# mehtas30/Software-Defined-Radio-Course-Project

Hardware: AMD Instinct MI355X
Metric: IQ Msamples/s (and x real-time) per GPU, mode-0 mono 2.4MS/s->48kS/s (higher is better)
Workload: dtype f32; 1 GPU; BASELINE configs[1]: mode-0 mono, 101-tap RF LPF + 10x decimate + FM demod + 51-tap audio LPF/5x decimate -> S16, 1 GiB synthetic u8 IQ per GPU (83,886 reference blocks), device-resident; mode=0, channels=1, rf_taps=101, stream_bytes_per_gpu=1073740800, blocks_per_gpu=83886, parallelism=streams x1 (one independent stream per GPU)

## Files before the change

### include/fmrx.h

```cpp
#ifndef FMRX_H
#define FMRX_H

#include <stddef.h>
#include <stdint.h>

#ifdef __cplusplus
extern "C" {
#endif

#define FMRX_OK 0
#define FMRX_EINVAL (-1)
#define FMRX_EHIP (-2)
#define FMRX_ENOMEM (-3)
#define FMRX_ESTATE (-4)

#define FMRX_STEREO 2
#define FMRX_MONO 1

typedef struct {
    int mode;
    int channels;
    int rf_taps;
    int bp_taps;
    int audio_taps;
// ... 256 lines not shown
int fmrx_rds_ext_init(fmrx_rds_ext* io);
int fmrx_rds_parse_blocks(fmrx_rds_ext* io, const fmrx_rds_block_rec* blocks, size_t n, uint64_t n_bits, int flush);
int fmrx_set_rds_sync(fmrx_ctx* ctx, int on);
int fmrx_rds_ext_get(const fmrx_ctx* ctx, int stream, fmrx_rds_ext* out);

int fmrx_fm_demod_arctan(fmrx_ctx* ctx, float* d_out, double* d_prev_phase, const float* d_i,
                         const float* d_q, int n);
int fmrx_estimate_psd(fmrx_ctx* ctx, const float* samples, size_t n, int freq_bins, float fs,
                      float* freq, float* psd_db);
int fmrx_psd_device(fmrx_ctx* ctx, const float* d_samples, size_t n, int freq_bins, float fs,
                    float* d_psd_db);

int fmrx_synth_host(uint64_t seed, int rf_fs, uint64_t first_pair, size_t n_pairs, uint8_t* out);
int fmrx_synth_device(fmrx_ctx* ctx, uint64_t seed, int rf_fs, uint64_t first_pair,
                      size_t n_pairs, uint8_t* d_out);
int fmrx_synth_device_streams(fmrx_ctx* ctx, const uint64_t* seeds, size_t n_seeds, int rf_fs,
                              uint64_t first_pair, size_t n_pairs, uint8_t* d_out, size_t stride_bytes);

int fmrx_test_pll_fallback(fmrx_ctx* ctx, int kind, const float* d_a, const float* d_b, size_t n,
                           float* d_out);

int fmrx_debug_mono_stamps(fmrx_ctx* ctx, unsigned long long* d_stamps, size_t n_workgroups, size_t* needed);

int fmrx_debug_pll_stats(fmrx_ctx* ctx, unsigned long long* d_counts);

int fmrx_debug_pll_redos(fmrx_ctx* ctx, unsigned* d_counts);

int fmrx_debug_stage_timing(fmrx_ctx* ctx, int op, double* ms, double* steps, long* launches, int n_kinds);

#define FMRX_KNOB_PLL_SPEC 0
#define FMRX_KNOB_PLL_SAT 1
#define FMRX_KNOB_PLL_PRED 2
#define FMRX_KNOB_PLL_PIPE 3
#define FMRX_KNOB_PLL_IDX 4
#define FMRX_KNOB_STEREO_CHUNKS 5
#define FMRX_KNOB_MONO_SPLIT 6
#define FMRX_KNOB_BPF_TILE 7
#define FMRX_KNOB_HALO_KERNEL 8
#define FMRX_KNOB_PLL_INJECT 9
#define FMRX_KNOB_PLL_PIPE_MISS 10
#define FMRX_KNOB_PLL_HINT_SKEW 11
#define FMRX_KNOB_PLL_CNT 12
#define FMRX_KNOB_PLL_STICK 13
#define FMRX_KNOB_STEREO_HEAD 14
#define FMRX_KNOB_STEREO_LEAD 15
#define FMRX_KNOB_AUDIO_DEFER 16
// ... 8 lines not shown
```

### software-defined-radio-course-project_amd/csrc/ctx.h

```cpp
#pragma once
#include <hip/hip_runtime.h>

#include <algorithm>
#include <cstdint>
#include <functional>
#include <limits>
#include <mutex>
#include <string>
#include <type_traits>
#include <utility>
#include <vector>

#include "../../include/fmrx.h"
#include "fmrx_internal.h"
#include "tuner.h"
#include "wide.h"

namespace fmrx {

int fail(int code, const char* fmt, ...);

#define HIPCHK(expr)                                                                   \
    do {                                                                               \
        hipError_t e_ = (expr);                                                        \
// ... 347 lines not shown
    HIPCHK(hipMemcpy(d.p, src, sizeof(float) * count, hipMemcpyHostToDevice));
    return 0;
}
inline size_t meter_frames(const fmrx_ctx* c, size_t n_blocks) {
    return n_blocks * c->geo.if_samples / ((size_t)kMeterWindows * (size_t)(c->geo.bp_fs / 1000));
}


int reset_state(fmrx_ctx* c);
int timing_begin(fmrx_ctx* c, hipStream_t st, TimingPair** ev);
inline int timing_end(TimingPair* ev, hipStream_t st) {
    if (ev) HIPCHK(hipEventRecord(ev->second, st));
    return 0;
}

int init_audio(fmrx_ctx* c);
int reset_audio(fmrx_ctx* c, const std::vector<float>& pll0);
int init_rds_front(fmrx_ctx* c);
int reset_rds_front(fmrx_ctx* c, const std::vector<float>& pll0);
int reset_deemph(fmrx_ctx* c);
int run_fused(fmrx_ctx* c, const uint8_t* d_iq, size_t n_blocks, int16_t* d_pcm, float* d_mono, float* d_demod,
              size_t demod_stride, int demod_hist, bool with_audio, size_t b0 = 0, size_t call_blocks = 0,
              hipStream_t st = nullptr, bool last = true);
int run_mono_audio(fmrx_ctx* c, const float* d_demod, size_t demod_stride, size_t n_if, int16_t* d_pcm, float* d_mono);
int run_stereo_audio(fmrx_ctx* c, size_t n_blocks, int16_t* d_pcm, float* d_mono, const float* src = nullptr);
int stereo_chunks(const fmrx_ctx* c, size_t n_blocks);
int run_stereo_pipelined(fmrx_ctx* c, const uint8_t* d_iq, size_t n_blocks, int16_t* d_pcm, float* d_mono, int K);
int run_rds(fmrx_ctx* c, const float* d_demod, size_t demod_stride, size_t n_if, float* d_out, float* d_nco,
            float* d_channel);
int ensure_demod(fmrx_ctx* c, size_t n_if);
int ensure_deemph_taps(fmrx_ctx* c);
inline int deemph_audio_fs(const fmrx_ctx* c) { return c->geo.if_fs / c->geo.audio_down; }

size_t rds_granule_blocks(const fmrx_ctx* c);
int check_rds_blocks(const fmrx_ctx* c, size_t n_blocks);
int init_rds_bits(fmrx_ctx* c);
int reset_rds_bits(fmrx_ctx* c);
int rds_decode_enqueue(fmrx_ctx* c, const float* d_demod, size_t demod_stride, size_t n_blocks);
int rds_decode_finish(fmrx_ctx* c);

void reset_rds_sync(fmrx_ctx* c);
int rds_sync_enqueue(fmrx_ctx* c, const uint8_t* d_bits, size_t n_bits);
int rds_sync_finish(fmrx_ctx* c);

void init_frames(fmrx_ctx* c);
int check_frame_blocks(const fmrx_ctx* c, size_t n_blocks, const char* who);
// ... 40 lines not shown
```

### software-defined-radio-course-project_amd/csrc/engine.cpp

```cpp
#include "ctx.h"

namespace fmrx {

static int grow_rows(fmrx_ctx* c, DevBuf<float>& buf, size_t& stride, size_t hist, size_t new_stride) {
    if (new_stride <= stride) return 0;
    const int ns = c->cfg.n_streams;
    DevBuf<float> nb;
    int rc = nb.ensure(new_stride * ns);
    if (rc) return rc;
    HIPCHK(hipMemsetAsync(nb.p, 0, sizeof(float) * nb.n, c->stream));
    if (buf.p) {
        HIPCHK(hipMemcpy2DAsync(nb.p, new_stride * sizeof(float), buf.p, stride * sizeof(float), hist * sizeof(float), ns,
                                hipMemcpyDeviceToDevice, c->stream));
        HIPCHK(hipStreamSynchronize(c->stream));
        buf.release();
    }
    buf = std::move(nb);
    stride = new_stride;
    return 0;
}

int init_audio(fmrx_ctx* c) {
    const fmrx_geometry_t& g = c->geo;
    const size_t ns = c->cfg.n_streams;
// ... 263 lines not shown
    L.stamps = c->diag.stamps;
    L.audio = with_audio ? 1 : 0;
    const bool fused_halo = (reinterpret_cast<uintptr_t>(L.iq) & 15) == 0 && L.stream_bytes % 16 == 0 &&
                            L.iq_stride % 16 == 0 && c->front.halo_bytes % 16 == 0 &&
                            c->knobs.halo_kernel != 1;
    L.halo_next = (last && fused_halo) ? c->front.halo.next() : nullptr;
    TimingPair* ev = nullptr;
    if ((rc = timing_begin(c, st, &ev))) return rc;
    const int st_t = (!with_audio && d_demod) ? c->diag.timer.begin(st) : -1;
    rc = launch_mono_fused(L, ns, c->geo.rf_taps, c->geo.rf_decim, c->geo.audio_up, c->geo.audio_down, c->taps.mono, st);
    c->diag.timer.end(st_t, kStFront, 0.0, st);
    if (rc != 0) return fail(rc == -1 ? FMRX_EINVAL : FMRX_EHIP, "fused kernel launch failed (%d)", rc);
    if ((rc = timing_end(ev, st))) return rc;
    if (with_audio) c->mono.stale = false;
    if (dx && (rc = run_quant_rows(c, dx, n_blocks * c->geo.audio_frames, d_pcm))) return rc;
    if (!last) return 0;
    if (!L.halo_next) {
        rc = launch_halo_update(d_iq, call_blocks * bb, c->front.halo.cur(), c->front.halo.next(),
                                c->front.halo_bytes, ns, st);
        if (rc != 0) return fail(FMRX_EHIP, "halo update failed");
    }
    c->front.halo.flip();
    return 0;
}

int run_mono_audio(fmrx_ctx* c, const float* d_demod, size_t demod_stride, size_t n_if,
                   int16_t* d_pcm, float* d_mono) {
    const int ns = c->cfg.n_streams;
    const int at = c->geo.audio_taps_total;
    const size_t na = n_if * c->geo.audio_up / c->geo.audio_down;
    PolyStreams P{};
    P.in = d_demod;
    P.in_stride = demod_stride;
    P.state = c->mono.hist.p;
    P.state_stride = c->mono.hist_len;
    P.coeff = c->taps.d_audio.p;
    P.taps = at;
    P.up = c->geo.audio_up;
    P.down = c->geo.audio_down;
    P.n_out = (int)na;
    float* dx = nullptr;
    int rc = quant_rows(c, na, d_mono, &dx);
    if (rc) return rc;
    P.out = dx ? dx : d_mono;
    P.out_stride = na;
    P.pcm = d_pcm;
// ... 220 lines not shown
```

### software-defined-radio-course-project_amd/csrc/mono_fused.hip

```cpp
#include <hip/hip_runtime.h>

#include <algorithm>
#include <cstdlib>

#include "dsp_device.h"
#include "mono_launch.h"

namespace fmrx {

namespace {

constexpr int kAudioTaps = 51;
constexpr int kAH = kAudioTaps - 1;

template <int T, int D, int AD, int NT, int R>
struct MonoCfg {
    static constexpr int S = R * D;
    static constexpr int G = (S % 4 == 2) ? 0 : 2;
    static constexpr int CIF = NT * R;
    static constexpr int P = CIF * D;
    static constexpr int H = T - 1;
    static constexpr int WH = T - 1 + D * (R - 1);
    static constexpr int slot(int b) { return b + G * (b / S); }
    static constexpr int XB = slot(H + P + 2) + 4;
    static constexpr int NLD = (P / 2 + NT - 1) / NT;
    static constexpr int LH0 = ((P - H) / 2) / NT;
    static constexpr int CAmax = (CIF + AD - 1) / AD;
    static constexpr int NG = (T + 1) / 2;
    static constexpr int na_for(int g) { return ((g * CIF + AD - 1) / AD + 1) / 2; }
    static constexpr int GA = na_for(3) <= NT ? 3 : na_for(2) <= NT ? 2 : 1;
    static constexpr int NA = na_for(GA);
    static constexpr int DX = AD * NA;
    static constexpr int DWI = DX + 50;
    static_assert(2 * DX >= GA * CIF, "every window sample has a slot");
    static_assert(T % 2 == 1, "odd tap count");
    static_assert(S % 2 == 0 && H % 2 == 0, "pair groups must stay 16-B aligned");
    static_assert(P % 2 == 0, "chunk must be whole dwords");
    static_assert(CAmax <= NT, "one audio output per thread per chunk");
};

__device__ inline uint32_t load4(const uint8_t* in, const uint8_t* halo, long long off,
                                 long long total, long long halo_bytes) {
    if (off >= 0) {
        if (off + 4 <= total) return *reinterpret_cast<const uint32_t*>(in + off);
        return 0x80808080u;
    }
    return *reinterpret_cast<const uint32_t*>(halo + (halo_bytes + off));
}

template <int K>
__device__ inline float sbyte(uint32_t w) {
    float f;
    if constexpr (K == 0)
        asm("v_cvt_f32_i32_sdwa %0, sext(%1) dst_sel:DWORD dst_unused:UNUSED_PAD src0_sel:BYTE_0" : "=v"(f) : "v"(w));
    else if constexpr (K == 1)
        asm("v_cvt_f32_i32_sdwa %0, sext(%1) dst_sel:DWORD dst_unused:UNUSED_PAD src0_sel:BYTE_1" : "=v"(f) : "v"(w));
    else if constexpr (K == 2)
        asm("v_cvt_f32_i32_sdwa %0, sext(%1) dst_sel:DWORD dst_unused:UNUSED_PAD src0_sel:BYTE_2" : "=v"(f) : "v"(w));
    else
        asm("v_cvt_f32_i32_sdwa %0, sext(%1) dst_sel:DWORD dst_unused:UNUSED_PAD src0_sel:BYTE_3" : "=v"(f) : "v"(w));
    return f;
}

template <int NT>
__device__ inline void chunk_sync() {
    if constexpr (NT == 64) {
        __builtin_amdgcn_fence(__ATOMIC_RELEASE, "wavefront");
        __builtin_amdgcn_wave_barrier();
        __builtin_amdgcn_fence(__ATOMIC_ACQUIRE, "wavefront");
    } else {
        __syncthreads();
    }
}

__device__ inline void mono_share(const MonoLaunch& L, int w, int n_chunks, int* stream, int* c0, int* c1) {
    if (L.older_share > 0) {
        const int half = L.segs / 2;
        const int H = (int)gridDim.x / 2;
        const int p = w < H ? w : w - H;
        const int s = p / half, q = p - s * half;
        const int p0 = (int)((long long)q * n_chunks / half), p1 = (int)((long long)(q + 1) * n_chunks / half);
        const int cut = p0 + (int)(((long long)(p1 - p0) * L.older_share) >> 10);
        *stream = s;
        *c0 = w < H ? p0 : cut;
        *c1 = w < H ? cut : p1;
        return;
    }
    *stream = w / L.segs;
    const int seg = w - *stream * L.segs;
    *c0 = (int)((long long)seg * n_chunks / L.segs);
    *c1 = (int)((long long)(seg + 1) * n_chunks / L.segs);
}

template <int T, int D, int AD, int NT, int R, int PD, int ABL = 0, int TR = 0, int AU = 1, int Z0 = 0>
__global__ void __launch_bounds__(NT) mono_fused_kernel(MonoLaunch L, MonoTaps taps) {
    using C = MonoCfg<T, D, AD, NT, R>;
    constexpr int CIF = C::CIF, P = C::P, H = C::H, S = C::S, G = C::G, NLD = C::NLD;
    constexpr int WH = C::WH, NG = C::NG;
    constexpr bool kShfl = NT == 64;
    static_assert(AU == 1 || ((long long)CIF * AU + AD - 1) / AD + 1 <= NT, "one audio output per thread");

    constexpr bool kWin = AU == 1;
    constexpr int GA = C::GA;
    __shared__ float4 xb4[C::XB / 2 + 1];
    __shared__ float2 dwi[kWin ? C::DWI : 1];
    __shared__ float dbuf[kWin ? 1 : 2][kWin ? 1 : kAH + CIF];
    __shared__ float2v pbuf[kShfl ? 1 : 2][kShfl ? 1 : NT + 1];
    __shared__ float2 ctab2[TR ? 1 : NG + 1];
    __shared__ float4 atab4[(kAudioTaps + 3) / 4];
    float* atab = reinterpret_cast<float*>(atab4);
    float* ctab = reinterpret_cast<float*>(ctab2);
    auto wput = [&](int s, float v) {
        if (s < C::DWI) dwi[s].x = v;
        if (s >= C::DX) dwi[s - C::DX].y = v;
    };

    const int tid = threadIdx.x;
    const long long n_if = L.n_if;
    const int n_chunks = (int)((n_if + CIF - 1) / CIF);
    if (L.halo_next) {
        const size_t words = L.halo_bytes / 16, total = words * (size_t)(gridDim.x / L.segs);
        for (size_t i = (size_t)blockIdx.x * NT + tid; i < total; i += (size_t)gridDim.x * NT) {
            const size_t s = i / words, j = i - s * words, v = L.stream_bytes + 16 * j;
            const uint4 w = v < L.halo_bytes ? *reinterpret_cast<const uint4*>(L.halo + s * L.halo_stride + v)
                                             : *reinterpret_cast<const uint4*>(L.iq + s * L.iq_stride + (v - L.halo_bytes));
            *reinterpret_cast<uint4*>(L.halo_next + s * L.halo_bytes + 16 * j) = w;
        }
    }
    int stream, c0, c1;
    mono_share(L, (int)blockIdx.x, n_chunks, &stream, &c0, &c1);
    const int c_full = (int)(L.stream_bytes / (2 * P));
    const int c_tail = n_if >= kAH ? (int)((n_if - kAH) / CIF) : -2;
    if (c0 >= c1) return;
    unsigned long long st_t0 = 0, st_r0 = 0;
    if constexpr ((ABL & 64) != 0) {
        st_t0 = __builtin_amdgcn_s_memtime();
        st_r0 = __builtin_amdgcn_s_memrealtime();
    }
    const long long n_audio = n_if * AU / AD;

    const uint8_t* in = L.iq + (size_t)stream * L.iq_stride;
    const uint8_t* halo = L.halo + (size_t)stream * L.halo_stride;
    const long long total = (long long)L.stream_bytes;
    const long long hb = (long long)L.halo_bytes;

    if constexpr (TR == 0)
        for (int i = tid; i < 2 * (NG + 1); i += NT) ctab[i] = (i >= 1 && i <= T) ? taps.rf[i - 1] : 0.0f;
    for (int i = tid; i < kAudioTaps; i += NT) atab[i] = taps.audio[i];

    for (int i = tid; i < H / 2; i += NT) {
        const uint32_t w = load4(in, halo, ((long long)(c0 - 1) * P - H + 2 * i) * 2, total, hb) ^ 0x80808080u;
        xb4[C::slot(2 * i) / 2] = make_float4(sbyte<0>(w), sbyte<1>(w), sbyte<2>(w), sbyte<3>(w));
    }
    uint32_t pf[NLD];
    auto fetch = [&](int cc) {
        if constexpr ((ABL & 16) != 0) {
#pragma unroll
// ... 4 lines not shown
        const int cl = cc < 0 ? 0 : (cc < c_full ? cc : c_full - 1);
        const uint32_t* src = reinterpret_cast<const uint32_t*>(in + (size_t)cl * (2 * P)) + tid;
#pragma unroll
        for (int l = 0; l < NLD; l++)
            if ((P / 2) % NT == 0 || tid + l * NT < P / 2) pf[l] = src[l * NT];
    };
    fetch(c0 - 1);

    float2 creg[TR ? NG : 1];
    if constexpr (TR != 0) {
#pragma unroll
        for (int j = 0; j < NG; j++) creg[j] = make_float2(j == 0 ? 0.0f : taps.rf[2 * j - 1], taps.rf[2 * j]);
    }
    int cur = 0;
    long long aq = (long long)(c0 - 1) * CIF / AD;
    int ar = (int)((long long)(c0 - 1) * CIF - aq * AD);
    float2v carry = {0.0f, 0.0f};
    float4 hist[NLD - C::LH0];
    int slot = -1;
    const int au_qt = AU > 1 ? tid * AD / AU : 0;
    const int au_rt = AU > 1 ? tid * AD - au_qt * AU : 0;
    long long wm0 = 0;
    int woff0 = 0;
    for (int c = c0 - 1; c < c1; c++) {
        if ((ABL & 16) == 0 && !(c >= 0 && c < c_full)) {
#pragma unroll
            for (int l = 0; l < NLD; l++) {
                const int u = tid + l * NT;
                if ((P / 2) % NT == 0 || u < P / 2) pf[l] = load4(in, halo, (long long)c * (2 * P) + 4LL * u, total, hb);
            }
        }
#pragma unroll
        for (int l = 0; l < NLD; l++) {
            const int u = tid + l * NT;
            if ((P / 2) % NT == 0 || u < P / 2) {
                const uint32_t w = pf[l] ^ 0x80808080u;
                if constexpr ((ABL & 32) != 0) {
                    asm volatile("" ::"v"(w));
                    continue;
                }
                const float4 f = (ABL & 8) != 0 ? make_float4(__uint_as_float(w), 0.f, 0.f, 0.f)
                                                : make_float4(sbyte<0>(w), sbyte<1>(w), sbyte<2>(w), sbyte<3>(w));
                xb4[C::slot(H + 2 * u) / 2] = f;
                if (l >= C::LH0) hist[l - C::LH0] = f;
            }
        }
// ... 62 lines not shown
            if (i >= 0 && ((P / 2) % NT == 0 || tid + l * NT < P / 2)) xb4[C::slot(2 * i) / 2] = hist[l - C::LH0];
        }
        float2v prev;
        if constexpr (!kShfl) {
            if (tid == 0) pbuf[cur ^ 1][0] = pbuf[cur][NT];
            prev = pbuf[cur][tid];
        } else {
            prev.x = __int_as_float(__builtin_amdgcn_update_dpp(__float_as_int(carry.x), __float_as_int(acc[R - 1].x),
                                                                0x138, 0xF, 0xF, false));
            prev.y = __int_as_float(__builtin_amdgcn_update_dpp(__float_as_int(carry.y), __float_as_int(acc[R - 1].y),
                                                                0x138, 0xF, 0xF, false));
            carry.x = __int_as_float(__builtin_amdgcn_readlane(__float_as_int(acc[R - 1].x), NT - 1));
            carry.y = __int_as_float(__builtin_amdgcn_readlane(__float_as_int(acc[R - 1].y), NT - 1));
        }
        float d[R];
#pragma unroll
        for (int r = 0; r < R; r++) {
            const float2v pv = r == 0 ? prev : acc[r - 1];
            if constexpr ((ABL & 4) != 0)
                d[r] = acc[r].x - pv.y;
            else
                d[r] = fm_demod_one(acc[r].x, acc[r].y, pv.x, pv.y);
        }
        const long long g0 = (long long)c * CIF + R * tid;
        if constexpr (kWin) {
            if (L.audio) {
#pragma unroll
                for (int r = 0; r < R; r++) {
                    const int jl = R * tid + r;
                    if (slot >= 0)
                        wput(kAH + slot * CIF + jl, d[r]);
                    else if (jl >= CIF - kAH)
                        wput(jl - (CIF - kAH), d[r]);
                }
            }
        } else {
#pragma unroll
            for (int r = 0; r < R; r++) {
                const int jl = R * tid + r;
                dbuf[cur][kAH + jl] = d[r];
                if (jl >= CIF - kAH) dbuf[cur ^ 1][jl - (CIF - kAH)] = d[r];
            }
        }
        if (c >= c0 && (L.demod || (L.demod_tail && c >= c_tail))) {
#pragma unroll
            for (int r = 0; r < R; r++) {
                const long long g = g0 + r;
                if (g < n_if) {
                    if (L.demod)
                        L.demod[(size_t)stream * L.demod_stride + L.demod_hist + g] = d[r];
                    if (L.demod_tail && g >= n_if - kAH)
                        L.demod_tail[(size_t)stream * L.demod_tail_stride + (g - (n_if - kAH))] = d[r];
                }
            }
        }
        chunk_sync<NT>();
        long long aq1 = aq + CIF / AD;
        int ar1 = ar + CIF % AD;
        if (ar1 >= AD) { ar1 -= AD; aq1++; }

        if constexpr (AU > 1) {
            if (L.audio && c >= c0) {
                const long long mlo = ((long long)c * CIF * AU + AD - 1) / AD;
                const long long mhi = ((long long)(c + 1) * CIF * AU + AD - 1) / AD;
                const long long m = mlo + tid;
                if (m < mhi && m < n_audio) {
                    const long long nb = mlo * AD;
                    const long long qb = nb / AU;
                    const int rb = (int)(nb - qb * AU);
                    const int rr = rb + au_rt;
                    const int wrap = rr >= AU ? 1 : 0;
                    const int k0 = rr - wrap * AU;
                    const int jl = (int)(qb - (long long)c * CIF) + au_qt + wrap;
                    const float* dw = &dbuf[cur][kAH + jl];
                    const float4* row = reinterpret_cast<const float4*>(L.audio_rows + (size_t)k0 * kAudioRow);
                    float4 cq[kAudioRow / 4];
                    float xv[kAudioTaps];
#pragma unroll
                    for (int i4 = 0; i4 < kAudioRow / 4; i4++) cq[i4] = row[i4];
#pragma unroll
                    for (int i = 0; i < kAudioTaps; i++) xv[i] = dw[-i];
                    __builtin_amdgcn_sched_barrier(0);
                    float a = 0.0f;
#pragma unroll
                    for (int i4 = 0; i4 < kAudioRow / 4; i4++) {
                        const float cv[4] = {cq[i4].x, cq[i4].y, cq[i4].z, cq[i4].w};
#pragma unroll
                        for (int e = 0; e < 4; e++) {
                            const int i = 4 * i4 + e;
                            if (i < kAudioTaps) {
                                const float p = cv[e] * xv[i];
                                a = a + p;
                            }
                        }
                    }
                    const size_t oi = (size_t)stream * (size_t)n_audio + (size_t)m;
                    L.pcm[oi] = quantize_s16(a);
                    if (L.mono) L.mono[oi] = a;
                }
            }
        } else if (L.audio && slot >= 0) {
            if (slot == 0) {
                wm0 = aq + (ar > 0);
                woff0 = ar > 0 ? AD - ar : 0;
            }
            if (slot == GA - 1 || c == c1 - 1) {
                long long mend = aq1 + (ar1 > 0);
                if (mend > n_audio) mend = n_audio;
                const long long nw = mend - wm0;
                if (tid < C::NA && tid < nw) {
                    const float2* base = dwi + woff0 + AD * tid;
                    float2v a2 = {0.0f, 0.0f};
                    constexpr int k0 = (Z0 & 2) ? 1 : 0, k1 = (ABL & 2) != 0 ? 1 : kAudioTaps, kAP = 16;
                    int zero_a;
                    asm volatile("v_mov_b32 %0, 0" : "=v"(zero_a));
                    const float4* at4 = atab4 + zero_a;
                    float4 tq[(kAudioTaps + 3) / 4];
#pragma unroll
                    for (int q = 0; q < (kAudioTaps + 3) / 4; q++) tq[q] = at4[q];
                    float2 xs[kAudioTaps];
#pragma unroll
                    for (int k = k0; k < k1 && k < k0 + kAP; k++) xs[k] = base[kAH - k];
#pragma unroll
                    for (int k = k0; k < k1; k++) {
                        if (k + kAP < k1) xs[k + kAP] = base[kAH - k - kAP];
                        const float4 t4 = tq[k / 4];
                        const float tk = (k & 3) == 0 ? t4.x : (k & 3) == 1 ? t4.y : (k & 3) == 2 ? t4.z : t4.w;
                        const float2v p = float2v{xs[k].x, xs[k].y} * tk;
                        a2 = a2 + p;
                    }
                    const size_t oi = (size_t)stream * (size_t)n_audio + (size_t)(wm0 + tid);
                    L.pcm[oi] = quantize_s16(a2.x);
                    if (L.mono) L.mono[oi] = a2.x;
                    if (tid + C::NA < nw) {
                        L.pcm[oi + C::NA] = quantize_s16(a2.y);
                        if (L.mono) L.mono[oi + C::NA] = a2.y;
                    }
                }
                if (slot == GA - 1) {
                    chunk_sync<NT>();
#pragma unroll
                    for (int r = 0; r < R; r++) {
                        const int jl = R * tid + r;
                        if (jl >= CIF - kAH) wput(jl - (CIF - kAH), d[r]);
                    }
                }
            }
        }
        cur ^= 1;
        aq = aq1;
        ar = ar1;
        if constexpr (kWin) slot = slot + 1 == GA ? 0 : slot + 1;
    }
    if constexpr ((ABL & 64) != 0) {
        const unsigned long long t1 = __builtin_amdgcn_s_memtime(), r1 = __builtin_amdgcn_s_memrealtime();
        const unsigned hw = __builtin_amdgcn_s_getreg(4 | (31 << 11));
        const unsigned xcc = __builtin_amdgcn_s_getreg(20 | (31 << 11));
        if (tid == 0 && L.stamps) {
            unsigned long long* o = L.stamps + 6 * ((size_t)blockIdx.x + tid);
            o[0] = st_t0;
            o[1] = t1;
            o[2] = st_r0;
            o[3] = r1;
            o[4] = hw;
            o[5] = xcc;
        }
    }
}

template <int T, int D, int AD, int NT, int R, int PD, int TR = 0, int AU = 1, int Z0 = 0>
int launch_variant(const MonoLaunch& L, int n_streams, const MonoTaps& taps, hipStream_t s) {
    hipLaunchKernelGGL((mono_fused_kernel<T, D, AD, NT, R, PD, 0, TR, AU, Z0>), dim3(n_streams * L.segs), dim3(NT), 0,
                       s, L, taps);
    return hipGetLastError() == hipSuccess ? 0 : -2;
}

bool tap0_zero(float h0) { return (__builtin_bit_cast(uint32_t, h0) & 0x7FFFFFFFu) == 0; }

struct Variant {
    int nt, r, pd, tr, wg_per_cu;
};
constexpr Variant kVariants[] = {{256, 3, 3, 0, 2}, {128, 3, 3, 0, 4}, {64, 3, 3, 0, 8}, {128, 5, 3, 0, 3},
                                 {256, 3, 5, 0, 2}, {64, 3, 3, 1, 8}, {64, 3, 4, 1, 8}};
constexpr int kDefaultVariant = 6;

int variant_index() {
    static int v = [] {
        const char* e = getenv("FMRX_MONO_VARIANT");
        const int i = e ? atoi(e) : kDefaultVariant;
        return (i >= 0 && i < (int)(sizeof kVariants / sizeof kVariants[0])) ? i : kDefaultVariant;
    }();
    return v;
}

}

size_t mono_halo_bytes(int rf_taps, int rf_decim, int ) {
    size_t pairs = 0;
    for (const Variant& v : kVariants) pairs = std::max(pairs, (size_t)v.nt * v.r * rf_decim);
    pairs += (size_t)(rf_taps - 1);
    return ((2 * pairs + 15) / 16) * 16 + 16;
}

long long mono_chunks(long long n_if, int , int rf_decim, int ) {
    const Variant v = kVariants[variant_index()];
    const long long cif = rf_decim == 9 ? 64 * 2 : (long long)v.nt * v.r;
    return (n_if + cif - 1) / cif;
}

int mono_wg_per_cu(int rf_decim) { return rf_decim == 9 ? 8 : kVariants[variant_index()].wg_per_cu; }

#ifdef FMRX_AB_ABLATE
int ablation() {
    static int a = [] {
        const char* e = getenv("FMRX_ABLATE");
        return e ? atoi(e) : 0;
    }();
    return a;
}
#endif

template <int ABL>
int launch_ablation(const MonoLaunch& L, int n_streams, const MonoTaps& taps, hipStream_t s) {
    hipLaunchKernelGGL((mono_fused_kernel<101, 10, 5, 64, 3, 4, ABL, 1>), dim3(n_streams * L.segs), dim3(64), 0,
                       s, L, taps);
    return hipGetLastError() == hipSuccess ? 0 : -2;
}

int launch_mono_fused(const MonoLaunch& L, int n_streams, int rf_taps, int rf_decim,
                      int audio_up, int audio_down, const MonoTaps& taps, hipStream_t s) {
// ... 68 lines not shown
```

### software-defined-radio-course-project_amd/csrc/mono_launch.h

```cpp
#pragma once
#include <hip/hip_runtime.h>
#include <stddef.h>
#include <stdint.h>

namespace fmrx {

constexpr int kMaxRfTaps = 256;

constexpr int kMaxAudioTaps = 64;
constexpr int kAudioRow = 52;

struct MonoTaps {
    float rf[kMaxRfTaps];
    float audio[kMaxAudioTaps];
};

struct MonoLaunch {
    const uint8_t* iq;
    const uint8_t* halo;
    int16_t* pcm;
    float* mono;
    float* demod;
    size_t demod_stride;
    int demod_hist;
    float* demod_tail;
    size_t demod_tail_stride;
    const float* audio_coeff;
    const float* audio_rows;
    size_t stream_bytes;
    size_t halo_bytes;
    long long n_if;
    int segs;
    int audio;
    unsigned long long* stamps;
    int older_share;
    uint8_t* halo_next;
    size_t iq_stride;
    size_t halo_stride;
};

size_t mono_halo_bytes(int rf_taps, int rf_decim, int audio_down);
long long mono_chunks(long long n_if, int rf_taps, int rf_decim, int audio_down);
int mono_wg_per_cu(int rf_decim);
int launch_mono_fused(const MonoLaunch& L, int n_streams, int rf_taps, int rf_decim,
                      int audio_up, int audio_down, const MonoTaps& taps, hipStream_t s);

}
```

### software-defined-radio-course-project_amd/csrc/prims_api.cpp

```cpp
#include <cmath>

#include "ctx.h"

using namespace fmrx;

extern "C" {

int fmrx_impulse_response_lpf(float* h, float fs, float fc, int taps, int gain) {
    if (!h || taps < 1) return fail(FMRX_EINVAL, "bad argument");
    design_lpf(h, fs, fc, taps, gain);
    return FMRX_OK;
}

int fmrx_impulse_response_bpf(float* h, float fs, float fb, float fe, int taps) {
    if (!h || taps < 1) return fail(FMRX_EINVAL, "bad argument");
    design_bpf(h, fs, fb, fe, taps);
    return FMRX_OK;
}

int fmrx_resample(fmrx_ctx* c, float* d_out, float* d_state, const float* d_in, int n_in,
                  const float* d_coeff, int taps, int up, int down, int* n_out) {
    CtxLock lock_(c);
    if (!c || !d_out || !d_state || !d_in || !d_coeff || taps < 1 || up < 1 || down < 1)
        return fail(FMRX_EINVAL, "bad argument");
// ... 163 lines not shown
    for (size_t k = 0; k < n_seeds; k++) synth_setup(seeds[k], rf_fs, &ps[k]);
    if ((rc = c->synth.params.ensure(sizeof(SynthParams) * n_seeds))) return rc;
    HIPCHK(hipMemcpyAsync(c->synth.params.p, ps.data(), sizeof(SynthParams) * n_seeds, hipMemcpyHostToDevice,
                          c->stream));
    if (launch_synth_streams(reinterpret_cast<const SynthParams*>(c->synth.params.p), (int)n_seeds,
                             c->synth.sintab.p, first_pair, n_pairs, d_out, stride_bytes, c->stream)) {
        (void)hipStreamSynchronize(c->stream);
        return fail(FMRX_EHIP, "synth launch failed");
    }
    HIPCHK(hipStreamSynchronize(c->stream));
    return FMRX_OK;
}

int fmrx_debug_mono_stamps(fmrx_ctx* c, unsigned long long* d_stamps, size_t n_workgroups, size_t* needed) {
    CtxLock lock_(c);
    if (!c) return fail(FMRX_EINVAL, "null context");
    if (needed) *needed = (size_t)c->cfg.n_streams * 256 * (size_t)mono_wg_per_cu(c->geo.rf_decim);
    if (d_stamps && needed && n_workgroups < *needed)
        return fail(FMRX_EINVAL, "stamp buffer holds %zu workgroups, up to %zu launch", n_workgroups, *needed);
    c->diag.stamps = d_stamps;
    return FMRX_OK;
}

int fmrx_debug_pll_redos(fmrx_ctx* c, unsigned* d_counts) {
    CtxLock lock_(c);
    if (!c) return fail(FMRX_EINVAL, "null context");
    c->diag.pll_redos = d_counts;
    return FMRX_OK;
}

int fmrx_debug_pll_stats(fmrx_ctx* c, unsigned long long* d_counts) {
    CtxLock lock_(c);
    if (!c) return fail(FMRX_EINVAL, "null context");
    c->diag.pll_stats = d_counts;
    return FMRX_OK;
}

}
```

### software-defined-radio-course-project_amd/fmrx.py

```python
from __future__ import annotations

import ctypes as C
import os
import re
from concurrent.futures import ThreadPoolExecutor
from contextlib import contextmanager
from typing import NamedTuple

import numpy as np

PKG_DIR = os.path.dirname(os.path.abspath(__file__))
REPO = os.path.dirname(PKG_DIR)
LIB_PATH = os.environ.get("FMRX_LIB_PATH") or os.path.join(PKG_DIR, "libfmrx.so")
HEADER = os.path.join(REPO, "include", "fmrx.h")

FMRX_OK, FMRX_EINVAL, FMRX_EHIP, FMRX_ENOMEM, FMRX_ESTATE = 0, -1, -2, -3, -4
MONO, STEREO = 1, 2
IQ_U8, IQ_S8, IQ_S16, IQ_F32 = 0, 1, 2, 3
IQ_DTYPES = {IQ_U8: np.dtype(np.uint8), IQ_S8: np.dtype(np.int8), IQ_S16: np.dtype("<i2"), IQ_F32: np.dtype("<f4")}


class FmrxError(RuntimeError):
    def __init__(self, code: int, msg: str):
        super().__init__(f"fmrx error {code}: {msg}")
# ... 296 lines not shown
    "fmrx_carrier_device": (C.c_int, [_vp, _vp, _sz, _vp]),
    "fmrx_carrier_accumulate": (C.c_int, [C.POINTER(CarrierReport), _vp, _sz]),
    "fmrx_afc_config_default": (C.c_int, [C.POINTER(AfcConfig)]),
    "fmrx_afc_decide": (C.c_int, [C.POINTER(CarrierReport), C.c_int, C.POINTER(AfcConfig), C.POINTER(AfcDecision)]),
    "fmrx_set_afc": (C.c_int, [_vp, C.POINTER(AfcConfig), C.c_int]),
    "fmrx_afc_get": (C.c_int, [_vp, C.c_int, C.POINTER(AfcStatus)]),
    "fmrx_synchronize": (C.c_int, [_vp]),
    "fmrx_stream": (_vp, [_vp]),
    "fmrx_kernel_timing": (C.c_int, [_vp, C.c_int, C.POINTER(C.c_double), C.POINTER(C.c_long)]),
    "fmrx_impulse_response_lpf": (C.c_int, [_fp, C.c_float, C.c_float, C.c_int, C.c_int]),
    "fmrx_impulse_response_bpf": (C.c_int, [_fp, C.c_float, C.c_float, C.c_float, C.c_int]),
    "fmrx_resample": (C.c_int, [_vp, _vp, _vp, _vp, C.c_int, _vp, C.c_int, C.c_int, C.c_int, C.POINTER(C.c_int)]),
    "fmrx_fm_demod": (C.c_int, [_vp, _vp, _vp, _vp, _vp, C.c_int]),
    "fmrx_pll": (C.c_int, [_vp, _vp, C.c_int, C.c_float, C.c_float, C.c_float, C.c_float, C.c_float, _vp]),
    "fmrx_mixer": (C.c_int, [_vp, _vp, _vp, _vp, C.c_int]),
    "fmrx_lr_extraction": (C.c_int, [_vp, _vp, _vp, _vp, _vp, C.c_int]),
    "fmrx_normalize_iq": (C.c_int, [_vp, _vp, _sz, _vp, _vp]),
    "fmrx_quantize": (C.c_int, [_vp, _vp, _sz, _vp]),
    "fmrx_synth_host": (C.c_int, [C.c_uint64, C.c_int, C.c_uint64, _sz, _vp]),
    "fmrx_synth_device": (C.c_int, [_vp, C.c_uint64, C.c_int, C.c_uint64, _sz, _vp]),
    "fmrx_synth_device_streams": (C.c_int, [_vp, _vp, _sz, C.c_int, C.c_uint64, _sz, _vp, _sz]),
    "fmrx_test_pll_fallback": (C.c_int, [_vp, C.c_int, _vp, _vp, _sz, _vp]),
    "fmrx_debug_mono_stamps": (C.c_int, [_vp, _vp, _sz, C.POINTER(_sz)]),
    "fmrx_debug_pll_stats": (C.c_int, [_vp, _vp]),
    "fmrx_debug_set_knob": (C.c_int, [_vp, C.c_int, C.c_double]),
    "fmrx_debug_pll_redos": (C.c_int, [_vp, _vp]),
    "fmrx_debug_stage_timing": (C.c_int, [_vp, C.c_int, C.POINTER(C.c_double), C.POINTER(C.c_double),
                                          C.POINTER(C.c_long), C.c_int]),
}

STAGES = ["front_end", "bandpass_pair", "pll_prep", "runner_lane", "runner_pred", "runner_sat", "runner_pipe20",
          "runner_pipe21", "runner_pipe22", "pll_check", "pll_tail", "pll_nco", "audio", "runner_idx17", "runner_idx18",
          "runner_idx19", "runner_cnt17", "runner_cnt18", "runner_cnt19", "runner_cnt20", "runner_cnt21", "runner_stick"]

KNOBS = {"pll_spec": 0, "pll_sat": 1, "pll_pred": 2, "pll_pipe": 3, "pll_idx": 4, "stereo_chunks": 5,
         "mono_split": 6, "bpf_tile": 7, "halo_kernel": 8, "pll_inject": 9, "pll_pipe_miss": 10,
         "pll_hint_skew": 11, "pll_cnt": 12, "pll_stick": 13, "stereo_head": 14,
         "stereo_lead": 15, "audio_defer": 16, "stereo_tail": 17}
REDO_RANGES = ["[2^17,2^20)", "[2^20,2^21)", "[2^21,2^22)", "[2^22,2^24]"]
REDO_SLOTS = 8
DEFAULT_KNOBS: dict = {}

_lib = None


def header_symbols() -> list[str]:
# ... 412 lines not shown
    route = _Route(mode, rf_taps, iq_format_of(iq), capture_decim, capture_rate)
    iq = _iq_flat(iq).reshape(-1)
    want = dict(rds=rds, probe=probe, blend=blend, afc=afc, quiet=quiet)
    with route.open(channels) as rx:
        stations = route.scan(rx, iq, **cfg)
    if not stations:
        return _stations_result([], _Run(np.zeros((0, 0), np.int16), [], [], [], quiets=[]), [], **want)
    lead, pulls = None, None
    if afc:
        lead, pulls = _afc_passes(route, iq, stations, probe)
    elif probe:
        lead = _leading_pass(route, iq, [s.offset_hz for s in stations], meter=True, measure=False)
    run = _grouped_decode(route, iq, [s.offset_hz for s in stations], channels, rds, lead.levels if lead else None,
                          rds_sync, blend, deemphasis_us, quiet)
    return _stations_result(stations, run, pulls, **want)


def synth_host(seed: int, rf_fs: int, first_pair: int, n_pairs: int) -> np.ndarray:
    out = np.zeros(2 * n_pairs, np.uint8)
    _check(lib().fmrx_synth_host(seed, rf_fs, first_pair, n_pairs, _np_ptr(out)))
    return out


class Receiver:

    def __init__(self, mode: int = 0, channels: int = MONO, rf_taps: int = 51, n_streams: int = 1,
                 device: int = 0, bp_taps: int = 51, audio_taps: int = 51, knobs: dict | None = None):
        self.cfg = default_config(mode, channels, rf_taps=rf_taps, n_streams=n_streams,
                                  device=device, bp_taps=bp_taps, audio_taps=audio_taps)
        self.geo = geometry(self.cfg)
        h = C.c_void_p()
        _check(lib().fmrx_create(C.byref(self.cfg), C.byref(h)))
        self.h = h
        self.n_streams = n_streams
        self.channels = channels
        for k, v in {**DEFAULT_KNOBS, **(knobs or {})}.items():
            self.set_knob(k, v)

    def set_knob(self, name: str, value: float) -> None:
        _check(lib().fmrx_debug_set_knob(self.h, KNOBS[name], float(value)))

    def close(self) -> None:
        if getattr(self, "h", None):
            lib().fmrx_destroy(self.h)
            self.h = None

# ... 460 lines not shown
    def pll(self, d_io, n, freq, fs, nco_scale, phase_adjust, norm_bw, d_state) -> None:
        _check(lib().fmrx_pll(self.h, d_io, n, freq, fs, nco_scale, phase_adjust, norm_bw, d_state))

    def mixer(self, d_out, d_a, d_b, n) -> None:
        _check(lib().fmrx_mixer(self.h, d_out, d_a, d_b, n))

    def lr_extraction(self, d_l, d_r, d_m, d_s, n) -> None:
        _check(lib().fmrx_lr_extraction(self.h, d_l, d_r, d_m, d_s, n))

    def normalize_iq(self, d_iq, n_pairs, d_i, d_q) -> None:
        _check(lib().fmrx_normalize_iq(self.h, d_iq, n_pairs, d_i, d_q))

    def quantize(self, d_x, n, d_out) -> None:
        _check(lib().fmrx_quantize(self.h, d_x, n, d_out))

    def test_pll_fallback(self, kind: int, d_a, d_b, n: int, d_out) -> None:
        _check(lib().fmrx_test_pll_fallback(self.h, kind, d_a, d_b, n, d_out))

    def debug_mono_stamps(self, d_stamps: int | None, n_workgroups: int = 0) -> int:
        need = _sz()
        _check(lib().fmrx_debug_mono_stamps(self.h, d_stamps, n_workgroups, C.byref(need)))
        return need.value

    def stage_timing(self, op: int) -> dict | None:
        n = len(STAGES)
        ms, steps, la = (C.c_double * n)(), (C.c_double * n)(), (C.c_long * n)()
        _check(lib().fmrx_debug_stage_timing(self.h, op, ms, steps, la, n))
        if op == 1:
            return None
        return {STAGES[k]: (ms[k], la[k], steps[k]) for k in range(n) if la[k]}

    def debug_pll_stats(self, d_counts: int | None) -> None:
        _check(lib().fmrx_debug_pll_stats(self.h, d_counts))

    def debug_pll_redos(self, d_counts) -> None:
        _check(lib().fmrx_debug_pll_redos(self.h, d_counts))


def build() -> None:
    import subprocess

    subprocess.run(["make", "-s", "-C", PKG_DIR, "-j8"], check=True)
```

Before: 969,900 MS/s.

## Add steady-state window fast path to fused mono kernel audio loop

```diff
diff --git a/include/fmrx.h b/include/fmrx.h
--- a/include/fmrx.h
+++ b/include/fmrx.h
@@ -302,6 +302,10 @@
 
 int fmrx_debug_mono_stamps(fmrx_ctx* ctx, unsigned long long* d_stamps, size_t n_workgroups, size_t* needed);
 
+int fmrx_debug_mono_plan(int n_chunks, int segs, int n_workgroups, int older_share, int w, int c_full, int c_tail,
+                         int ga, int flags, int out[5]);
+int fmrx_debug_mono_grid(fmrx_ctx* ctx, size_t n_blocks, int out[6]);
+
 int fmrx_debug_pll_stats(fmrx_ctx* ctx, unsigned long long* d_counts);
 
 int fmrx_debug_pll_redos(fmrx_ctx* ctx, unsigned* d_counts);
diff --git a/software-defined-radio-course-project_amd/csrc/ctx.h b/software-defined-radio-course-project_amd/csrc/ctx.h
--- a/software-defined-radio-course-project_amd/csrc/ctx.h
+++ b/software-defined-radio-course-project_amd/csrc/ctx.h
@@ -393,6 +393,7 @@
 int run_fused(fmrx_ctx* c, const uint8_t* d_iq, size_t n_blocks, int16_t* d_pcm, float* d_mono, float* d_demod,
               size_t demod_stride, int demod_hist, bool with_audio, size_t b0 = 0, size_t call_blocks = 0,
               hipStream_t st = nullptr, bool last = true);
+void mono_call_grid(const fmrx_ctx* c, size_t n_blocks, int out[6]);
 int run_mono_audio(fmrx_ctx* c, const float* d_demod, size_t demod_stride, size_t n_if, int16_t* d_pcm, float* d_mono);
 int run_stereo_audio(fmrx_ctx* c, size_t n_blocks, int16_t* d_pcm, float* d_mono, const float* src = nullptr);
 int stereo_chunks(const fmrx_ctx* c, size_t n_blocks);
diff --git a/software-defined-radio-course-project_amd/csrc/engine.cpp b/software-defined-radio-course-project_amd/csrc/engine.cpp
--- a/software-defined-radio-course-project_amd/csrc/engine.cpp
+++ b/software-defined-radio-course-project_amd/csrc/engine.cpp
@@ -309,6 +309,14 @@
     }
     c->front.halo.flip();
     return 0;
+}
+
+void mono_call_grid(const fmrx_ctx* c, size_t n_blocks, int out[6]) {
+    const long long n_if = (long long)(n_blocks * c->geo.if_samples);
+    out[0] = mono_segments(c, n_if);
+    out[1] = mono_older_share(c, out[0]);
+    mono_plan_geometry(n_if, n_blocks * c->geo.block_bytes, c->geo.rf_decim, c->geo.audio_down, &out[2], &out[3], &out[4],
+                       &out[5]);
 }
 
 int run_mono_audio(fmrx_ctx* c, const float* d_demod, size_t demod_stride, size_t n_if,
diff --git a/software-defined-radio-course-project_amd/csrc/mono_fused.hip b/software-defined-radio-course-project_amd/csrc/mono_fused.hip
--- a/software-defined-radio-course-project_amd/csrc/mono_fused.hip
+++ b/software-defined-radio-course-project_amd/csrc/mono_fused.hip
@@ -2,6 +2,7 @@
 
 #include <algorithm>
 #include <cstdlib>
+#include <type_traits>
 
 #include "dsp_device.h"
 #include "mono_launch.h"
@@ -12,6 +13,11 @@
 
 constexpr int kAudioTaps = 51;
 constexpr int kAH = kAudioTaps - 1;
+
+constexpr int window_chunks(int cif, int ad, int nt) {
+    const int na3 = ((3 * cif + ad - 1) / ad + 1) / 2, na2 = ((2 * cif + ad - 1) / ad + 1) / 2;
+    return na3 <= nt ? 3 : na2 <= nt ? 2 : 1;
+}
 
 template <int T, int D, int AD, int NT, int R>
 struct MonoCfg {
@@ -28,7 +34,7 @@
     static constexpr int CAmax = (CIF + AD - 1) / AD;
     static constexpr int NG = (T + 1) / 2;
     static constexpr int na_for(int g) { return ((g * CIF + AD - 1) / AD + 1) / 2; }
-    static constexpr int GA = na_for(3) <= NT ? 3 : na_for(2) <= NT ? 2 : 1;
+    static constexpr int GA = window_chunks(CIF, AD, NT);
     static constexpr int NA = na_for(GA);
     static constexpr int DX = AD * NA;
     static constexpr int DWI = DX + 50;
@@ -74,22 +80,7 @@
 }
 
 __device__ inline void mono_share(const MonoLaunch& L, int w, int n_chunks, int* stream, int* c0, int* c1) {
-    if (L.older_share > 0) {
-        const int half = L.segs / 2;
-        const int H = (int)gridDim.x / 2;
-        const int p = w < H ? w : w - H;
-        const int s = p / half, q = p - s * half;
-        const int p0 = (int)((long long)q * n_chunks / half), p1 = (int)((long long)(q + 1) * n_chunks / half);
-        const int cut = p0 + (int)(((long long)(p1 - p0) * L.older_share) >> 10);
-        *stream = s;
-        *c0 = w < H ? p0 : cut;
-        *c1 = w < H ? cut : p1;
-        return;
-    }
-    *stream = w / L.segs;
-    const int seg = w - *stream * L.segs;
-    *c0 = (int)((long long)seg * n_chunks / L.segs);
-    *c1 = (int)((long long)(seg + 1) * n_chunks / L.segs);
+    mono_range(L.older_share, L.segs, (int)gridDim.x, w, n_chunks, stream, c0, c1);
 }
 
 template <int T, int D, int AD, int NT, int R, int PD, int ABL = 0, int TR = 0, int AU = 1, int Z0 = 0>
@@ -129,10 +120,11 @@
     }
     int stream, c0, c1;
     mono_share(L, (int)blockIdx.x, n_chunks, &stream, &c0, &c1);
-    const int c_full = (int)(L.stream_bytes / (2 * P));
-    const int c_tail = n_if >= kAH ? (int)((n_if - kAH) / CIF) : -2;
+    const int c_full = mono_c_full(L.stream_bytes, P);
+    const int c_tail = mono_c_tail(n_if, CIF);
     if (c0 >= c1) return;
     unsigned long long st_t0 = 0, st_r0 = 0;
+    unsigned steady_windows = 0;
     if constexpr ((ABL & 64) != 0) {
         st_t0 = __builtin_amdgcn_s_memtime();
         st_r0 = __builtin_amdgcn_s_memrealtime();
@@ -183,6 +175,18 @@
     const int au_rt = AU > 1 ? tid * AD - au_qt * AU : 0;
     long long wm0 = 0;
     int woff0 = 0;
+    int s_left = 0, sl = 0, s_ar = 0;
+    int16_t* s_pcm = nullptr;
+    if constexpr (kWin) {
+        const MonoPlan plan = mono_plan(c0, c1, c_full, c_tail, GA, mono_plan_flags(L));
+        if (plan.windows > 0) {
+            const long long q0 = (long long)c0 * CIF / AD;
+            s_ar = (int)((long long)c0 * CIF - q0 * AD);
+            s_pcm = L.pcm + ((size_t)stream * (size_t)n_audio + (size_t)(q0 + (s_ar > 0)));
+            s_left = GA * plan.windows;
+            steady_windows = (unsigned)plan.windows;
+        }
+    }
     for (int c = c0 - 1; c < c1; c++) {
         if ((ABL & 16) == 0 && !(c >= 0 && c < c_full)) {
 #pragma unroll
@@ -291,92 +295,151 @@
             else
                 d[r] = fm_demod_one(acc[r].x, acc[r].y, pv.x, pv.y);
         }
-        const long long g0 = (long long)c * CIF + R * tid;
-        if constexpr (kWin) {
-            if (L.audio) {
+        bool fire = false, wlast = false;
+        int nw = 0;
+        int16_t* po = nullptr;
+        float* pm = nullptr;
+        if (kWin && s_left > 0 && c >= c0) {
+            int zero_w;
+            asm volatile("v_mov_b32 %0, 0" : "=v"(zero_w));
+            const int tb = R * tid + zero_w;
+            auto put = [&](auto kslot) {
+                constexpr int k = decltype(kslot)::value;
+                constexpr int lo = kAH + k * CIF, hi = lo + CIF - 1;
+#pragma unroll
+                for (int r = 0; r < R; r++) {
+                    const int s = lo + tb + r;
+                    if (hi < C::DWI || (lo < C::DWI && s < C::DWI)) dwi[s].x = d[r];
+                    if (lo >= C::DX || (hi >= C::DX && s >= C::DX)) dwi[s - C::DX].y = d[r];
+                }
+            };
+            if (sl == 0) {
+                put(std::integral_constant<int, 0>{});
+            } else if constexpr (GA > 2) {
+                if (sl == 1)
+                    put(std::integral_constant<int, 1>{});
+                else
+                    put(std::integral_constant<int, 2>{});
+            } else if constexpr (GA > 1) {
+                put(std::integral_constant<int, 1>{});
+            }
+            chunk_sync<NT>();
+            if (sl == GA - 1) {
+                const int e = s_ar + GA * CIF;
+                fire = wlast = true;
+                woff0 = s_ar > 0 ? AD - s_ar : 0;
+                nw = (e + AD - 1) / AD - (s_ar > 0 ? 1 : 0);
+                po = s_pcm;
+                s_pcm += nw;
+                s_ar = e % AD;
+            }
+            sl = sl + 1 == GA ? 0 : sl + 1;
+            cur ^= 1;
+            if (--s_left == 0) {
+                aq = (long long)(c + 1) * CIF / AD;
+                ar = (int)((long long)(c + 1) * CIF - aq * AD);
+            }
+        } else {
+            const long long g0 = (long long)c * CIF + R * tid;
+            if constexpr (kWin) {
+                if (L.audio) {
+#pragma unroll
+                    for (int r = 0; r < R; r++) {
+                        const int jl = R * tid + r;
+                        if (slot >= 0)
+                            wput(kAH + slot * CIF + jl, d[r]);
+                        else if (jl >= CIF - kAH)
+                            wput(jl - (CIF - kAH), d[r]);
+                    }
+                }
+            } else {
 #pragma unroll
                 for (int r = 0; r < R; r++) {
                     const int jl = R * tid + r;
-                    if (slot >= 0)
-                        wput(kAH + slot * CIF + jl, d[r]);
-                    else if (jl >= CIF - kAH)
-                        wput(jl - (CIF - kAH), d[r]);
-                }
-            }
-        } else {
-#pragma unroll
-            for (int r = 0; r < R; r++) {
-                const int jl = R * tid + r;
-                dbuf[cur][kAH + jl] = d[r];
-                if (jl >= CIF - kAH) dbuf[cur ^ 1][jl - (CIF - kAH)] = d[r];
-            }
-        }
-        if (c >= c0 && (L.demod || (L.demod_tail && c >= c_tail))) {
-#pragma unroll
-            for (int r = 0; r < R; r++) {
-                const long long g = g0 + r;
-                if (g < n_if) {
-                    if (L.demod)
-                        L.demod[(size_t)stream * L.demod_stride + L.demod_hist + g] = d[r];
-                    if (L.demod_tail && g >= n_if - kAH)
-                        L.demod_tail[(size_t)stream * L.demod_tail_stride + (g - (n_if - kAH))] = d[r];
-                }
-            }
-        }
-        chunk_sync<NT>();
-        long long aq1 = aq + CIF / AD;
-        int ar1 = ar + CIF % AD;
-        if (ar1 >= AD) { ar1 -= AD; aq1++; }
-
-        if constexpr (AU > 1) {
-            if (L.audio && c >= c0) {
-                const long long mlo = ((long long)c * CIF * AU + AD - 1) / AD;
-                const long long mhi = ((long long)(c + 1) * CIF * AU + AD - 1) / AD;
-                const long long m = mlo + tid;
-                if (m < mhi && m < n_audio) {
-                    const long long nb = mlo * AD;
-                    const long long qb = nb / AU;
-                    const int rb = (int)(nb - qb * AU);
-                    const int rr = rb + au_rt;
-                    const int wrap = rr >= AU ? 1 : 0;
-                    const int k0 = rr - wrap * AU;
-                    const int jl = (int)(qb - (long long)c * CIF) + au_qt + wrap;
-                    const float* dw = &dbuf[cur][kAH + jl];
-                    const float4* row = reinterpret_cast<const float4*>(L.audio_rows + (size_t)k0 * kAudioRow);
-                    float4 cq[kAudioRow / 4];
-                    float xv[kAudioTaps];
-#pragma unroll
-                    for (int i4 = 0; i4 < kAudioRow / 4; i4++) cq[i4] = row[i4];
-#pragma unroll
-                    for (int i = 0; i < kAudioTaps; i++) xv[i] = dw[-i];
-                    __builtin_amdgcn_sched_barrier(0);
-                    float a = 0.0f;
-#pragma unroll
-                    for (int i4 = 0; i4 < kAudioRow / 4; i4++) {
-                        const float cv[4] = {cq[i4].x, cq[i4].y, cq[i4].z, cq[i4].w};
-#pragma unroll
-                        for (int e = 0; e < 4; e++) {
-                            const int i = 4 * i4 + e;
-                            if (i < kAudioTaps) {
-                                const float p = cv[e] * xv[i];
-                                a = a + p;
+                    dbuf[cur][kAH + jl] = d[r];
+                    if (jl >= CIF - kAH) dbuf[cur ^ 1][jl - (CIF - kAH)] = d[r];
+                }
+            }
+            if (c >= c0 && (L.demod || (L.demod_tail && c >= c_tail))) {
+#pragma unroll
+                for (int r = 0; r < R; r++) {
+                    const long long g = g0 + r;
+                    if (g < n_if) {
+                        if (L.demod)
+                            L.demod[(size_t)stream * L.demod_stride + L.demod_hist + g] = d[r];
+                        if (L.demod_tail && g >= n_if - kAH)
+                            L.demod_tail[(size_t)stream * L.demod_tail_stride + (g - (n_if - kAH))] = d[r];
+                    }
+                }
+            }
+            chunk_sync<NT>();
+            long long aq1 = aq + CIF / AD;
+            int ar1 = ar + CIF % AD;
+            if (ar1 >= AD) { ar1 -= AD; aq1++; }
+
+            if constexpr (AU > 1) {
+                if (L.audio && c >= c0) {
+                    const long long mlo = ((long long)c * CIF * AU + AD - 1) / AD;
+                    const long long mhi = ((long long)(c + 1) * CIF * AU + AD - 1) / AD;
+                    const long long m = mlo + tid;
+                    if (m < mhi && m < n_audio) {
+                        const long long nb = mlo * AD;
+                        const long long qb = nb / AU;
+                        const int rb = (int)(nb - qb * AU);
+                        const int rr = rb + au_rt;
+                        const int wrap = rr >= AU ? 1 : 0;
+                        const int k0 = rr - wrap * AU;
+                        const int jl = (int)(qb - (long long)c * CIF) + au_qt + wrap;
+                        const float* dw = &dbuf[cur][kAH + jl];
+                        const float4* row = reinterpret_cast<const float4*>(L.audio_rows + (size_t)k0 * kAudioRow);
+                        float4 cq[kAudioRow / 4];
+                        float xv[kAudioTaps];
+#pragma unroll
+                        for (int i4 = 0; i4 < kAudioRow / 4; i4++) cq[i4] = row[i4];
+#pragma unroll
+                        for (int i = 0; i < kAudioTaps; i++) xv[i] = dw[-i];
+                        __builtin_amdgcn_sched_barrier(0);
+                        float a = 0.0f;
+#pragma unroll
+                        for (int i4 = 0; i4 < kAudioRow / 4; i4++) {
+                            const float cv[4] = {cq[i4].x, cq[i4].y, cq[i4].z, cq[i4].w};
+#pragma unroll
+                            for (int e = 0; e < 4; e++) {
+                                const int i = 4 * i4 + e;
+                                if (i < kAudioTaps) {
+                                    const float p = cv[e] * xv[i];
+                                    a = a + p;
+                                }
                             }
                         }
+                        const size_t oi = (size_t)stream * (size_t)n_audio + (size_t)m;
+                        L.pcm[oi] = quantize_s16(a);
+                        if (L.mono) L.mono[oi] = a;
                     }
-                    const size_t oi = (size_t)stream * (size_t)n_audio + (size_t)m;
-                    L.pcm[oi] = quantize_s16(a);
-                    if (L.mono) L.mono[oi] = a;
-                }
-            }
-        } else if (L.audio && slot >= 0) {
-            if (slot == 0) {
-                wm0 = aq + (ar > 0);
-                woff0 = ar > 0 ? AD - ar : 0;
-            }
-            if (slot == GA - 1 || c == c1 - 1) {
-                long long mend = aq1 + (ar1 > 0);
-                if (mend > n_audio) mend = n_audio;
-                const long long nw = mend - wm0;
+                }
+            } else if (L.audio && slot >= 0) {
+                if (slot == 0) {
+                    wm0 = aq + (ar > 0);
+                    woff0 = ar > 0 ? AD - ar : 0;
+                }
+                if (slot == GA - 1 || c == c1 - 1) {
+                    long long mend = aq1 + (ar1 > 0);
+                    if (mend > n_audio) mend = n_audio;
+                    const size_t oi = (size_t)stream * (size_t)n_audio + (size_t)wm0;
+                    fire = true;
+                    wlast = slot == GA - 1;
+                    nw = (int)(mend - wm0);
+                    po = L.pcm + oi;
+                    pm = L.mono ? L.mono + oi : nullptr;
+                }
+            }
+            cur ^= 1;
+            aq = aq1;
+            ar = ar1;
+            if constexpr (kWin) slot = slot + 1 == GA ? 0 : slot + 1;
+        }
+        if constexpr (kWin) {
+            if (fire) {
                 if (tid < C::NA && tid < nw) {
                     const float2* base = dwi + woff0 + AD * tid;
                     float2v a2 = {0.0f, 0.0f};
@@ -398,15 +461,14 @@
                         const float2v p = float2v{xs[k].x, xs[k].y} * tk;
                         a2 = a2 + p;
                     }
-                    const size_t oi = (size_t)stream * (size_t)n_audio + (size_t)(wm0 + tid);
-                    L.pcm[oi] = quantize_s16(a2.x);
-                    if (L.mono) L.mono[oi] = a2.x;
+                    po[tid] = quantize_s16(a2.x);
+                    if (pm) pm[tid] = a2.x;
                     if (tid + C::NA < nw) {
-                        L.pcm[oi + C::NA] = quantize_s16(a2.y);
-                        if (L.mono) L.mono[oi + C::NA] = a2.y;
+                        po[tid + C::NA] = quantize_s16(a2.y);
+                        if (pm) pm[tid + C::NA] = a2.y;
                     }
                 }
-                if (slot == GA - 1) {
+                if (wlast) {
                     chunk_sync<NT>();
 #pragma unroll
                     for (int r = 0; r < R; r++) {
@@ -416,10 +478,6 @@
                 }
             }
         }
-        cur ^= 1;
-        aq = aq1;
-        ar = ar1;
-        if constexpr (kWin) slot = slot + 1 == GA ? 0 : slot + 1;
     }
     if constexpr ((ABL & 64) != 0) {
         const unsigned long long t1 = __builtin_amdgcn_s_memtime(), r1 = __builtin_amdgcn_s_memrealtime();
@@ -431,7 +489,7 @@
             o[1] = t1;
             o[2] = st_r0;
             o[3] = r1;
-            o[4] = hw;
+            o[4] = hw | ((unsigned long long)steady_windows << 32);
             o[5] = xcc;
         }
     }
@@ -475,6 +533,16 @@
     const Variant v = kVariants[variant_index()];
     const long long cif = rf_decim == 9 ? 64 * 2 : (long long)v.nt * v.r;
     return (n_if + cif - 1) / cif;
+}
+
+void mono_plan_geometry(long long n_if, size_t stream_bytes, int rf_decim, int audio_down, int* n_chunks, int* c_full,
+                        int* c_tail, int* ga) {
+    const Variant v = kVariants[variant_index()];
+    const int cif = v.nt * v.r;
+    *n_chunks = (int)((n_if + cif - 1) / cif);
+    *c_full = mono_c_full(stream_bytes, cif * rf_decim);
+    *c_tail = mono_c_tail(n_if, cif);
+    *ga = window_chunks(cif, audio_down, v.nt);
 }
 
 int mono_wg_per_cu(int rf_decim) { return rf_decim == 9 ? 8 : kVariants[variant_index()].wg_per_cu; }
diff --git a/software-defined-radio-course-project_amd/csrc/mono_launch.h b/software-defined-radio-course-project_amd/csrc/mono_launch.h
--- a/software-defined-radio-course-project_amd/csrc/mono_launch.h
+++ b/software-defined-radio-course-project_amd/csrc/mono_launch.h
@@ -39,8 +39,49 @@
     size_t halo_stride;
 };
 
+__host__ __device__ inline void mono_range(int older_share, int segs, int n_wg, int w, int n_chunks, int* stream,
+                                           int* c0, int* c1) {
+    if (older_share > 0) {
+        const int half = segs / 2;
+        const int H = n_wg / 2;
+        const int p = w < H ? w : w - H;
+        const int s = p / half, q = p - s * half;
+        const int p0 = (int)((long long)q * n_chunks / half), p1 = (int)((long long)(q + 1) * n_chunks / half);
+        const int cut = p0 + (int)(((long long)(p1 - p0) * older_share) >> 10);
+        *stream = s;
+        *c0 = w < H ? p0 : cut;
+        *c1 = w < H ? cut : p1;
+        return;
+    }
+    *stream = w / segs;
+    const int seg = w - *stream * segs;
+    *c0 = (int)((long long)seg * n_chunks / segs);
+    *c1 = (int)((long long)(seg + 1) * n_chunks / segs);
+}
+
+__host__ __device__ inline int mono_c_full(size_t stream_bytes, int pairs) { return (int)(stream_bytes / (size_t)(2 * pairs)); }
+__host__ __device__ inline int mono_c_tail(long long n_if, int cif) { return n_if >= 50 ? (int)((n_if - 50) / cif) : -2; }
+constexpr int kMonoPlanAudio = 1, kMonoPlanDemod = 2, kMonoPlanMono = 4;
+struct MonoPlan {
+    int first;
+    int windows;
+};
+__host__ __device__ inline MonoPlan mono_plan(int c0, int c1, int c_full, int c_tail, int ga, int flags) {
+    MonoPlan p{c0, 0};
+    if (flags != kMonoPlanAudio || c0 < 0 || ga < 1) return p;
+    int hi = c1 < c_full ? c1 : c_full;
+    if (c_tail < hi) hi = c_tail;
+    if (hi > c0) p.windows = (hi - c0) / ga;
+    return p;
+}
+__host__ __device__ inline int mono_plan_flags(const MonoLaunch& L) {
+    return (L.audio ? kMonoPlanAudio : 0) | (L.demod ? kMonoPlanDemod : 0) | (L.mono ? kMonoPlanMono : 0);
+}
+
 size_t mono_halo_bytes(int rf_taps, int rf_decim, int audio_down);
 long long mono_chunks(long long n_if, int rf_taps, int rf_decim, int audio_down);
+void mono_plan_geometry(long long n_if, size_t stream_bytes, int rf_decim, int audio_down, int* n_chunks, int* c_full,
+                        int* c_tail, int* ga);
 int mono_wg_per_cu(int rf_decim);
 int launch_mono_fused(const MonoLaunch& L, int n_streams, int rf_taps, int rf_decim,
                       int audio_up, int audio_down, const MonoTaps& taps, hipStream_t s);
diff --git a/software-defined-radio-course-project_amd/csrc/prims_api.cpp b/software-defined-radio-course-project_amd/csrc/prims_api.cpp
--- a/software-defined-radio-course-project_amd/csrc/prims_api.cpp
+++ b/software-defined-radio-course-project_amd/csrc/prims_api.cpp
@@ -209,6 +209,25 @@
     return FMRX_OK;
 }
 
+int fmrx_debug_mono_plan(int n_chunks, int segs, int n_workgroups, int older_share, int w, int c_full, int c_tail, int ga,
+                         int flags, int out[5]) {
+    if (!out || n_chunks < 0 || segs < 1 || n_workgroups < segs || w < 0 || w >= n_workgroups || ga < 1 ||
+        (older_share > 0 && (segs & 1)))
+        return fail(FMRX_EINVAL, "bad argument");
+    mono_range(older_share, segs, n_workgroups, w, n_chunks, &out[0], &out[1], &out[2]);
+    const MonoPlan p = mono_plan(out[1], out[2], c_full, c_tail, ga, flags);
+    out[3] = p.first;
+    out[4] = p.windows;
+    return FMRX_OK;
+}
+
+int fmrx_debug_mono_grid(fmrx_ctx* c, size_t n_blocks, int out[6]) {
+    CtxLock lock_(c);
+    if (!c || !out || n_blocks == 0) return fail(FMRX_EINVAL, "bad argument");
+    mono_call_grid(c, n_blocks, out);
+    return FMRX_OK;
+}
+
 int fmrx_debug_pll_redos(fmrx_ctx* c, unsigned* d_counts) {
     CtxLock lock_(c);
     if (!c) return fail(FMRX_EINVAL, "null context");
diff --git a/software-defined-radio-course-project_amd/fmrx.py b/software-defined-radio-course-project_amd/fmrx.py
--- a/software-defined-radio-course-project_amd/fmrx.py
+++ b/software-defined-radio-course-project_amd/fmrx.py
@@ -342,6 +342,8 @@
     "fmrx_synth_device_streams": (C.c_int, [_vp, _vp, _sz, C.c_int, C.c_uint64, _sz, _vp, _sz]),
     "fmrx_test_pll_fallback": (C.c_int, [_vp, C.c_int, _vp, _vp, _sz, _vp]),
     "fmrx_debug_mono_stamps": (C.c_int, [_vp, _vp, _sz, C.POINTER(_sz)]),
+    "fmrx_debug_mono_plan": (C.c_int, [C.c_int] * 9 + [C.POINTER(C.c_int)]),
+    "fmrx_debug_mono_grid": (C.c_int, [_vp, _sz, C.POINTER(C.c_int)]),
     "fmrx_debug_pll_stats": (C.c_int, [_vp, _vp]),
     "fmrx_debug_set_knob": (C.c_int, [_vp, C.c_int, C.c_double]),
     "fmrx_debug_pll_redos": (C.c_int, [_vp, _vp]),
@@ -800,6 +802,16 @@
     return out
 
 
+MONO_PLAN_AUDIO, MONO_PLAN_DEMOD, MONO_PLAN_MONO = 1, 2, 4
+
+
+def debug_mono_plan(n_chunks: int, segs: int, n_workgroups: int, older_share: int, w: int, c_full: int, c_tail: int,
+                    ga: int = 3, flags: int = MONO_PLAN_AUDIO) -> dict:
+    out = (C.c_int * 5)()
+    _check(lib().fmrx_debug_mono_plan(n_chunks, segs, n_workgroups, older_share, w, c_full, c_tail, ga, flags, out))
+    return dict(zip(("stream", "c0", "c1", "first", "windows"), out))
+
+
 class Receiver:
 
     def __init__(self, mode: int = 0, channels: int = MONO, rf_taps: int = 51, n_streams: int = 1,
@@ -1306,6 +1318,11 @@
         _check(lib().fmrx_debug_mono_stamps(self.h, d_stamps, n_workgroups, C.byref(need)))
         return need.value
 
+    def debug_mono_grid(self, n_blocks: int) -> dict:
+        out = (C.c_int * 6)()
+        _check(lib().fmrx_debug_mono_grid(self.h, n_blocks, out))
+        return dict(zip(("segs", "older_share", "n_chunks", "c_full", "c_tail", "ga"), out))
+
     def stage_timing(self, op: int) -> dict | None:
         n = len(STAGES)
         ms, steps, la = (C.c_double * n)(), (C.c_double * n)(), (C.c_long * n)()
```

Result: no change. 970,700 MS/s (median of 6 runs) (+0.1%).
